# Viasat/nhd

Hardware: AMD Instinct MI355X
Metric: pod-placement filter-and-score throughput (pod x node fit-and-score evaluations/s; placement decisions/s under commit semantics in mode_b) (higher is better)
Workload: dtype u64 bitmaps + int32 table look-ups (f64 NIC arithmetic in the request digest)

## Files before the change

nhd_amd/csrc/set_states.h:

```cpp
#pragma once
#include "winner_map.h"

#include <unordered_map>
#include <vector>

namespace nhdfit {

struct SetStates {
    const uint64_t* info;
    const uint32_t* next;
    const uint32_t* asc;
    uint32_t n;
};

NHD_HD uint32_t st_key(uint64_t w, uint32_t j) { return (uint32_t)(w >> (3 * j)) & 7u; }
NHD_HD uint32_t st_count(uint64_t w) { return (uint32_t)(w >> 24) & 15u; }
NHD_HD uint32_t st_pick(uint64_t w) { return (uint32_t)(w >> 28) & 7u; }
NHD_HD uint32_t st_present(uint64_t w) { return (uint32_t)(w >> 32) & 0xFFu; }

NHD_HD uint32_t st_intersect(const SetStates& T, uint32_t a, uint32_t b) {
    const uint64_t wa = T.info[a], wb = T.info[b];
    const bool swap = st_count(wb) > st_count(wa);
    const uint64_t iter = swap ? wa : wb;
    const uint32_t probe = st_present(swap ? wb : wa);
    uint32_t out = 0;
    for (uint32_t j = 0; j < st_count(iter); ++j) {
        const uint32_t k = st_key(iter, j);
        if (probe >> k & 1) out = T.next[out * 8 + k];
    }
    return out;
}

NHD_HD uint32_t choose_g3(const SetStates& T, const AscEntry* asc, uint32_t sg_mask, uint32_t sc_mask, uint32_t nic_codes) {
    sg_mask &= 0xFFu; sc_mask &= 0xFFFFu; nic_codes &= 0xFFu;
    const uint32_t sgS = T.asc[sg_mask], cS = T.asc[nic_codes];
    const SmallSet sc = ss_from_asc(asc, 4, 2, sc_mask);
    const uint64_t wsg = T.info[sgS];
    uint32_t a = 0, b = 0;
    for (uint32_t j = 0; j < st_count(wsg); ++j) a = T.next[a * 8 + st_key(wsg, j)];
    for (int i = ss_next(sc, 0); i >= 0; i = ss_next(sc, i + 1)) b = T.next[b * 8 + ((uint32_t)ss_key(sc, i) >> 1)];
    const uint32_t abc = st_intersect(T, st_intersect(T, a, b), cS);
    const uint64_t wabc = T.info[abc];
    if (st_count(wabc) == 0) return 0;
    const uint32_t gcode = st_count(wabc) < st_count(wsg) ? st_pick(wabc) : st_pick(wsg);
    int ccode = -1;
    for (int i = ss_next(sc, 0); i >= 0 && ccode < 0; i = ss_next(sc, i + 1)) {
        const int k = ss_key(sc, i);
        if ((uint32_t)(k >> 1) == gcode) ccode = k;
    }
    return choose_result_word(ccode >= 0, gcode, ccode);
}

inline void build_set_states(std::vector<uint64_t>& info, std::vector<uint32_t>& next, std::vector<uint32_t>& asc) {
    struct Key {
        uint32_t used; int mask; uint64_t k0, k1;
        bool operator==(const Key& o) const { return used == o.used && mask == o.mask && k0 == o.k0 && k1 == o.k1; }
    };
    struct Hash {
        size_t operator()(const Key& k) const {
            uint64_t h = k.used * 0x9E3779B97F4A7C15ull ^ (uint64_t)k.mask;
            h = (h ^ k.k0) * 0xC2B2AE3D27D4EB4Full;
            h = (h ^ k.k1) * 0x165667B19E3779F9ull;
            return (size_t)(h ^ (h >> 29));
        }
    };
    std::unordered_map<Key, uint32_t, Hash> ids;
    std::vector<SmallSet> sets;
    auto intern = [&](const SmallSet& s) -> uint32_t {
        const Key key{s.used, s.mask, s.k0, s.k1};
        auto it = ids.find(key);
        if (it != ids.end()) return it->second;
        const uint32_t id = (uint32_t)sets.size();
        ids.emplace(key, id);
        sets.push_back(s);
        return id;
    };
    intern(ss_make(3, 2));
    next.clear();
    for (uint32_t s = 0; s < sets.size(); ++s) {
        for (int k = 0; k < 8; ++k) {
            const SmallSet cur = sets[s];
            const uint32_t t = (cur.present >> k & 1) ? s : intern(ss_add(cur, k));
            next.push_back(t);
        }
    }
    info.resize(sets.size());
    for (uint32_t s = 0; s < sets.size(); ++s) {
        const SmallSet& x = sets[s];
        uint64_t w = 0;
        uint32_t j = 0;
        for (int i = ss_next(x, 0); i >= 0; i = ss_next(x, i + 1)) w |= (uint64_t)ss_key(x, i) << (3 * j++);
        w |= (uint64_t)j << 24;
        if (j) w |= (uint64_t)(pick_gpu_tuple<SmallOps>(x, 3, 2) & 7) << 28;
        w |= (uint64_t)(x.present & 0xFFu) << 32;
        info[s] = w;
    }
    asc.assign(256, 0);
    for (uint32_t subset = 0; subset < 256; ++subset) {
        uint32_t s = 0;
        for (int k = 0; k < 8; ++k)
            if (subset >> k & 1) s = next[s * 8 + k];
        asc[subset] = s;
    }
// ... 4 lines not shown
```

nhd_amd/csrc/step_map.h:

```cpp
__device__ __forceinline__ bool load_winner(const MapArgs& a, uint32_t p, WinnerState& w, uint32_t& i) {
    const unsigned long long s = a.score[p];
    if (!s) return false;
    const uint64_t gi = NHDFIT_SCORE_INDEX(s);
    if (gi < a.global_base || gi >= a.global_base + a.n) return false;
    i = (uint32_t)(gi - a.global_base);
    const nhdfit_plane0 q0 = a.p0[i];
    const nhdfit_plane1 q1 = a.p1[i];
    const nhdfit_plane2 q2 = a.p2[i];
    w.d = a.det + i;
    w.U = w.d->numa_nodes;
    w.smt = (q2.flags & NHDFIT_NF_SMT) != 0;
    w.free_c[0] = popc64(q0.t0[0] & q1.t1[0]);
    w.free_c[1] = popc64(q0.t0[1] & q1.t1[1]);
    w.free_g[0] = popc32(q2.gpu_free & ~q2.gpu_numa1);
    w.free_g[1] = popc32(q2.gpu_free & q2.gpu_numa1);
    w.caps = a.caps;
    return true;
}

struct ShapeArgs {
    unsigned long long* keys;
    uint32_t* result;
    int32_t* slot_of_pod;
    uint32_t* count;
    const AscEntry* asc;
    const uint8_t* choose_tab;
    SetStates st;
};

__global__ __launch_bounds__(256) void k_build_choose(const AscEntry* asc, uint8_t* table) {
    const uint32_t e = blockIdx.x * 256 + threadIdx.x;
    if (e < kChooseEntries) table[e] = choose_entry_build(asc, e);
}

__global__ __launch_bounds__(256) void k_build_asc(AscEntry* table) {
    const uint32_t e = blockIdx.x * 256 + threadIdx.x;
    if (e >= kAscEntries) return;
    const int len = e >= kAscOffset[4] ? 4 : e >= kAscOffset[3] ? 3 : e >= kAscOffset[2] ? 2 : 1;
    table[e] = asc_entry_build(len, e - kAscOffset[len]);
}


__device__ __forceinline__ unsigned long long shfl64(unsigned long long v, int lane) {
    return ((unsigned long long)(uint32_t)__shfl((int)(v >> 32), lane, 64) << 32) | (uint32_t)__shfl((int)(uint32_t)v, lane, 64);
}

struct PaddedDet { nhdfit_detail d; uint32_t pad; };
struct StagedNode {
    int32_t node;
    uint32_t free_c[2], free_g[2];
    uint16_t sig_numa[2], sig_pci[2];
    uint32_t smt, U;
};
struct MapStage {
    PaddedReq* req; PaddedDet* det; StagedNode* w; nhdfit_mapping* map; double* caps;
};
template <int THREADS>
constexpr size_t map_lds_bytes() {
    constexpr size_t pods = THREADS / 4;
    return lds_slice(pods * sizeof(PaddedReq)) + lds_slice(pods * sizeof(PaddedDet)) + lds_slice(pods * sizeof(StagedNode)) +
           lds_slice(pods * sizeof(nhdfit_mapping)) + lds_slice(NHDFIT_MAX_CLASSES * sizeof(double));
}
constexpr uint32_t kStLdsStates = 384;
constexpr size_t kStLdsBytes = lds_slice(kStLdsStates * sizeof(uint64_t)) + lds_slice((size_t)kStLdsStates * 8 * sizeof(uint32_t)) + lds_slice(256 * sizeof(uint32_t));
template <int THREADS>
constexpr size_t map_tile_lds_bytes() { return map_lds_bytes<THREADS>() + kStLdsBytes; }
template <int THREADS>
__device__ __forceinline__ MapStage stage_winners(const MapArgs& a, uint32_t pod0, uint8_t* lds) {
    constexpr uint32_t PODS = THREADS / 4;
    MapStage s;
    s.req = carve<PaddedReq>(lds, PODS);
    s.det = carve<PaddedDet>(lds, PODS);
    s.w = carve<StagedNode>(lds, PODS);
    s.map = carve<nhdfit_mapping>(lds, PODS);
    s.caps = carve<double>(lds, NHDFIT_MAX_CLASSES);
    const uint32_t tid = threadIdx.x;
    constexpr uint32_t kParts = sizeof(nhdfit_req) / 16;
    const uint32_t live = pod0 < a.P ? (a.P - pod0 < PODS ? a.P - pod0 : PODS) : 0u;
    {
        const uint4* src = reinterpret_cast<const uint4*>(a.reqs + pod0);
        for (uint32_t c = tid; c < PODS * kParts; c += THREADS) {
            const uint32_t j = c / kParts;
            const uint4 v = j < live ? src[c] : make_uint4(0u, 0u, 0u, 0u);
            uint32_t* dst = reinterpret_cast<uint32_t*>(&s.req[j]) + (c % kParts) * 4;
            dst[0] = v.x; dst[1] = v.y; dst[2] = v.z; dst[3] = v.w;
        }
    }
    if (tid < NHDFIT_MAX_CLASSES) s.caps[tid] = a.caps[tid];
    if (tid < PODS) {
        StagedNode n;
        n.node = -1;
        n.free_c[0] = n.free_c[1] = n.free_g[0] = n.free_g[1] = 0; n.smt = 0; n.U = 1;
        n.sig_numa[0] = n.sig_numa[1] = n.sig_pci[0] = n.sig_pci[1] = 0;
        const unsigned long long sc = tid < live ? a.score[pod0 + tid] : 0ull;
        if (sc) {
            const uint64_t gi = NHDFIT_SCORE_INDEX(sc);
            if (gi >= a.global_base && gi < a.global_base + a.n) {
                const uint32_t i = (uint32_t)(gi - a.global_base);
                const nhdfit_plane0 q0 = a.p0[i];
                const nhdfit_plane1 q1 = a.p1[i];
                const nhdfit_plane2 q2 = a.p2[i];
                const nhdfit_plane3 q3 = a.p3[i];
                n.node = (int32_t)i;
                n.smt = (q2.flags & NHDFIT_NF_SMT) != 0;
                n.free_c[0] = popc64(q0.t0[0] & q1.t1[0]); n.free_c[1] = popc64(q0.t0[1] & q1.t1[1]);
                n.free_g[0] = popc32(q2.gpu_free & ~q2.gpu_numa1); n.free_g[1] = popc32(q2.gpu_free & q2.gpu_numa1);
                n.sig_numa[0] = q3.sig_numa[0]; n.sig_numa[1] = q3.sig_numa[1];
                n.sig_pci[0] = q3.sig_pci[0]; n.sig_pci[1] = q3.sig_pci[1];
            }
        }
        s.w[tid] = n;
    }
    __syncthreads();
    constexpr uint32_t kDetParts = sizeof(nhdfit_detail) / 16;
    for (uint32_t c = tid; c < PODS * kDetParts; c += THREADS) {
        const uint32_t j = c / kDetParts, part = c % kDetParts;
        const int32_t i = s.w[j].node;
        if (i >= 0) {
            const uint4 v = reinterpret_cast<const uint4*>(a.det + i)[part];
            uint32_t* dst = reinterpret_cast<uint32_t*>(&s.det[j]) + part * 4;
            dst[0] = v.x; dst[1] = v.y; dst[2] = v.z; dst[3] = v.w;
        }
    }
    __syncthreads();
    return s;
}
__device__ __forceinline__ WinnerState staged_state(const MapStage& s, uint32_t j) {
    WinnerState w;
    w.d = &s.det[j].d;
    w.U = s.det[j].d.numa_nodes;
    w.smt = s.w[j].smt != 0;
    w.free_c[0] = (int)s.w[j].free_c[0]; w.free_c[1] = (int)s.w[j].free_c[1];
    w.free_g[0] = (int)s.w[j].free_g[0]; w.free_g[1] = (int)s.w[j].free_g[1];
    w.caps = s.caps;
    return w;
}

template <int THREADS>
__device__ __forceinline__ void role_shapes(const MapArgs& a, const ShapeArgs& h, uint32_t blk, uint8_t* lds) {
    constexpr uint32_t PODS = THREADS / 4;
    const uint32_t pod0 = blk * PODS;
    const MapStage st = stage_winners<THREADS>(a, pod0, lds);
    if (threadIdx.x >= PODS) return;
    const uint32_t j = threadIdx.x, p = pod0 + j, tile = p >> 6, lane = threadIdx.x & 63;
    if (tile * 64 >= a.P) return;
    int32_t slot = -1;
    unsigned long long key = 0;
    const nhdfit_req& rq = st.req[j].r;
    if (p < a.P && rq.n_groups <= 3 && st.w[j].node >= 0) {
        const WinnerState w = staged_state(st, j);
        nhdfit_plane3 q3;
        q3.groups = 0;
        q3.sig_numa[0] = st.w[j].sig_numa[0]; q3.sig_numa[1] = st.w[j].sig_numa[1];
        q3.sig_pci[0] = st.w[j].sig_pci[0]; q3.sig_pci[1] = st.w[j].sig_pci[1];
        const uint32_t bits = nic_assignment_bits(a.tabs + (size_t)tile * a.pitch, a.L[a.tile_wcls[tile]], lane,
                                                  rq.map_type == NHDFIT_MAP_PCI, q3);
        const uint32_t codes = nic_codes_from_table_bits(bits, (int)rq.n_groups, w.U);
        uint32_t sg, sc;
        candidate_masks(rq, w, sg, sc);
        if (sg && sc && codes) {
            if (h.choose_tab && choose_tabulated((int)rq.n_groups, w.U))
                slot = -2 - (int32_t)choose_from_table(h.choose_tab, (int)rq.n_groups, sg, sc, codes);
            else
                key = shape_key((int)rq.n_groups, w.U, sg, sc, codes);
        }
    }
    unsigned long long todo = __ballot(key != 0ull);
    uint32_t nd = 0;
    while (todo) {
        const int leader = __builtin_ctzll(todo);
        const unsigned long long k = shfl64(key, leader);
        if ((int)lane == leader) h.keys[tile * 64 + nd] = k;
        if (key == k) slot = (int32_t)(tile * 64 + nd);
        todo &= ~__ballot(key == k);
        ++nd;
    }
    if (lane == 0) h.count[tile] = nd;
    if (p < a.P) h.slot_of_pod[p] = slot;
}

__device__ __forceinline__ void role_choose(const ShapeArgs& h, uint32_t w, uint32_t waves, uint32_t tiles) {
    const uint32_t S = waves / tiles ? waves / tiles : 1u;
    if (w >= S * tiles) return;
    const uint32_t tile = w % tiles, sub = w / tiles;
    const uint32_t count = (uint32_t)__builtin_amdgcn_readfirstlane((int)h.count[tile]);
    for (uint32_t j = sub; j < count; j += S) {
        const uint32_t k = tile * 64 + j;
        const unsigned long long kv = h.keys[k];
        const unsigned long long key = ((unsigned long long)(uint32_t)__builtin_amdgcn_readfirstlane((int)(kv >> 32)) << 32) |
                                       (uint32_t)__builtin_amdgcn_readfirstlane((int)(uint32_t)kv);
        const int G = (int)(key & 3), U = (int)((key >> 2) & 1) + 1;
        uint32_t gcode = 0;
        int ccode = -1;
        if (h.st.info && G == 3 && U == 2) {
            h.result[k] = choose_g3(h.st, h.asc, (uint32_t)(key >> 3) & 0xFF, (uint32_t)(key >> 19) & 0xFFFF, (uint32_t)(key >> 11) & 0xFF);
            continue;
        }
        const bool ok = choose_tuples<SmallOps>(G, U, (uint32_t)(key >> 3) & 0xFF, (uint32_t)(key >> 19) & 0xFFFF,
                                                (uint32_t)(key >> 11) & 0xFF, gcode, ccode, h.asc);
        h.result[k] = ((uint32_t)ok << 8) | ((gcode & 7u) << 4) | ((uint32_t)ccode & 15u);
    }
}

__device__ __forceinline__ void role_choose_lanes(const ShapeArgs& h, uint32_t tile, uint32_t tiles) {
    if (tile >= tiles) return;
    const uint32_t lane = threadIdx.x & 63;
    const uint32_t count = (uint32_t)__builtin_amdgcn_readfirstlane((int)h.count[tile]);
    const uint32_t k = tile * 64 + lane;
    unsigned long long key = 0;
    bool generic = false;
    if (lane < count) {
        key = h.keys[k];
        const int G = (int)(key & 3), U = (int)((key >> 2) & 1) + 1;
        if (h.st.info && G == 3 && U == 2)
            h.result[k] = choose_g3(h.st, h.asc, (uint32_t)(key >> 3) & 0xFF, (uint32_t)(key >> 19) & 0xFFFF, (uint32_t)(key >> 11) & 0xFF);
        else
            generic = true;
    }
    unsigned long long todo = __ballot(generic);
    while (todo) {
        const int j = __builtin_ctzll(todo);
        todo &= todo - 1;
        const unsigned long long kv = shfl64(key, j);
        if (lane == 0) {
            const unsigned long long kk = ((unsigned long long)(uint32_t)__builtin_amdgcn_readfirstlane((int)(kv >> 32)) << 32) |
                                          (uint32_t)__builtin_amdgcn_readfirstlane((int)(uint32_t)kv);
            const int G = (int)(kk & 3), U = (int)((kk >> 2) & 1) + 1;
            uint32_t gcode = 0;
            int ccode = -1;
            const bool ok = choose_tuples<SmallOps>(G, U, (uint32_t)(kk >> 3) & 0xFF, (uint32_t)(kk >> 19) & 0xFFFF,
                                                    (uint32_t)(kk >> 11) & 0xFF, gcode, ccode, h.asc);
            h.result[tile * 64 + j] = ((uint32_t)ok << 8) | ((gcode & 7u) << 4) | ((uint32_t)ccode & 15u);
        }
    }
}

template <int THREADS>
__device__ __forceinline__ void role_finish(const MapArgs& a, const ShapeArgs& h, uint32_t blk, uint8_t* lds) {
    constexpr uint32_t PODS = THREADS / 4;
    const uint32_t pod0 = blk * PODS;
    const MapStage st = stage_winners<THREADS>(a, pod0, lds);
    const uint32_t j = threadIdx.x, p = pod0 + j;
    if (j < PODS) {
        nhdfit_mapping& m = st.map[j];
        memset(&m, 0, sizeof(m));
        const nhdfit_req& rq = st.req[j].r;
        if (p < a.P && rq.n_groups <= 3) {
            const int32_t slot = h.slot_of_pod[p];
            if (slot != -1) {
                const uint32_t res = slot >= 0 ? h.result[slot] : (uint32_t)(-2 - slot);
                if ((res >> 8 & 1) && st.w[j].node >= 0) finish_mapping(rq, staged_state(st, j), (res >> 4) & 7u, (int)(res & 15u), m);
            }
        }
    }
    __syncthreads();
    const uint32_t live = pod0 < a.P ? (a.P - pod0 < PODS ? a.P - pod0 : PODS) : 0u;
    constexpr uint32_t kWords = sizeof(nhdfit_mapping) / 4;
    const uint32_t* src = reinterpret_cast<const uint32_t*>(st.map);
    uint32_t* dst = reinterpret_cast<uint32_t*>(a.out + pod0);
    for (uint32_t c = threadIdx.x; c < live * kWords; c += THREADS)
        if (st.req[c / kWords].r.n_groups <= 3) dst[c] = src[c];
}

template <int THREADS, bool LONE = false>
__device__ __forceinline__ void map_one_tile(const MapArgs& a, const ShapeArgs& h, uint32_t wcls, uint8_t* lds, const LoneMasks* lone = nullptr,
                                             uint32_t tile = 0, unsigned long long* clk = nullptr) {
    const unsigned long long t_blk = kTuning && clk ? (unsigned long long)wall_clock64() : 0ull;
    auto lap = [&](int k) { if (kTuning && clk && threadIdx.x == 0) atomicMax(&clk[k], (unsigned long long)wall_clock64() - t_blk); };
    static_assert(THREADS / 4 == kTile, "the pods of the tile are one wavefront");
    const uint32_t pod0 = tile * kTile;
    SetStates lst = h.st;
    if (h.st.info && h.st.n <= kStLdsStates) {
        uint8_t* q = lds + map_lds_bytes<THREADS>();
        uint64_t* l_info = carve<uint64_t>(q, kStLdsStates);
        uint32_t* l_next = carve<uint32_t>(q, (size_t)kStLdsStates * 8);
        uint32_t* l_asc = carve<uint32_t>(q, 256);
        for (uint32_t i = threadIdx.x; i < h.st.n; i += THREADS) l_info[i] = h.st.info[i];
        for (uint32_t i = threadIdx.x; i < h.st.n * 8; i += THREADS) l_next[i] = h.st.next[i];
        for (uint32_t i = threadIdx.x; i < 256; i += THREADS) l_asc[i] = h.st.asc[i];
        lst = SetStates{l_info, l_next, l_asc, h.st.n};
    }
    const MapStage st = stage_winners<THREADS>(a, pod0, lds);
    lap(0);
    const uint32_t j = threadIdx.x;
    if (j < (uint32_t)kTile) {
        const uint32_t lane = j;
        nhdfit_mapping& m = st.map[j];
        memset(&m, 0, sizeof(m));
        const nhdfit_req& rq = st.req[j].r;
        const bool live = pod0 + j < a.P && rq.n_groups <= 3 && st.w[j].node >= 0;
        int32_t slot = -1;
        unsigned long long key = 0;
        if (live) {
            const WinnerState w = staged_state(st, j);
            nhdfit_plane3 q3;
            q3.groups = 0;
            q3.sig_numa[0] = st.w[j].sig_numa[0]; q3.sig_numa[1] = st.w[j].sig_numa[1];
            q3.sig_pci[0] = st.w[j].sig_pci[0]; q3.sig_pci[1] = st.w[j].sig_pci[1];
            uint32_t bits;
            if constexpr (LONE) bits = lone_nic_bits(*lone, rq.map_type == NHDFIT_MAP_PCI, q3);
            else bits = nic_assignment_bits(a.tabs + (size_t)tile * a.pitch, a.L[wcls], lane, rq.map_type == NHDFIT_MAP_PCI, q3);
            const uint32_t codes = nic_codes_from_table_bits(bits, (int)rq.n_groups, w.U);
            uint32_t sg, sc;
            candidate_masks(rq, w, sg, sc);
            if (sg && sc && codes) {
                if (h.choose_tab && choose_tabulated((int)rq.n_groups, w.U))
                    slot = -2 - (int32_t)choose_from_table(h.choose_tab, (int)rq.n_groups, sg, sc, codes);
                else
                    key = shape_key((int)rq.n_groups, w.U, sg, sc, codes);
            }
        }
        lap(1);
        unsigned long long todo = __ballot(key != 0ull), mine = 0;
        uint32_t nd = 0;
        while (todo) {
            const int leader = __builtin_ctzll(todo);
            const unsigned long long k = shfl64(key, leader);
            if (lane == nd) mine = k;
            if (key == k) slot = (int32_t)nd;
            todo &= ~__ballot(key == k);
            ++nd;
        }
        lap(2);
        uint32_t res = 0;
        bool generic = false;
        if (lane < nd) {
            const int G = (int)(mine & 3), U = (int)((mine >> 2) & 1) + 1;
            if (lst.info && G == 3 && U == 2)
                res = choose_g3(lst, h.asc, (uint32_t)(mine >> 3) & 0xFF, (uint32_t)(mine >> 19) & 0xFFFF, (uint32_t)(mine >> 11) & 0xFF);
            else
                generic = true;
        }
        lap(3);
        unsigned long long gtodo = __ballot(generic);
        while (gtodo) {
            const int jj = __builtin_ctzll(gtodo);
            gtodo &= gtodo - 1;
            const unsigned long long kv = shfl64(mine, jj);
            uint32_t r = 0;
            if (lane == 0) {
                const unsigned long long kk = ((unsigned long long)(uint32_t)__builtin_amdgcn_readfirstlane((int)(kv >> 32)) << 32) |
                                              (uint32_t)__builtin_amdgcn_readfirstlane((int)(uint32_t)kv);
                const int G = (int)(kk & 3), U = (int)((kk >> 2) & 1) + 1;
                uint32_t gcode = 0;
                int ccode = -1;
                const bool ok = choose_tuples<SmallOps>(G, U, (uint32_t)(kk >> 3) & 0xFF, (uint32_t)(kk >> 19) & 0xFFFF,
                                                        (uint32_t)(kk >> 11) & 0xFF, gcode, ccode, h.asc);
                r = ((uint32_t)ok << 8) | ((gcode & 7u) << 4) | ((uint32_t)ccode & 15u);
            }
            r = (uint32_t)__shfl((int)r, 0, 64);
            if ((int)lane == jj) res = r;
        }
        lap(4);
        const uint32_t got = (uint32_t)__shfl((int)res, slot >= 0 ? slot : 0, 64);
        if (live && slot != -1) {
            const uint32_t rr = slot >= 0 ? got : (uint32_t)(-2 - slot);
            if (rr >> 8 & 1) finish_mapping(rq, staged_state(st, j), (rr >> 4) & 7u, (int)(rr & 15u), m);
        }
        lap(5);
    }
    __syncthreads();
    const uint32_t livep = pod0 < a.P ? (a.P - pod0 < (uint32_t)kTile ? a.P - pod0 : (uint32_t)kTile) : 0u;
    constexpr uint32_t kWords = sizeof(nhdfit_mapping) / 4;
    const uint32_t* src = reinterpret_cast<const uint32_t*>(st.map);
    uint32_t* dst = reinterpret_cast<uint32_t*>(a.out + pod0);
    for (uint32_t c = threadIdx.x; c < livep * kWords; c += THREADS)
        if (st.req[c / kWords].r.n_groups <= 3) dst[c] = src[c];
}

constexpr int kDrainSteps = 3;
struct DrainArgs {
    uint32_t nsteps, tiles;
    MapArgs m[kDrainSteps];
    ShapeArgs h;
    unsigned long long* clk;
};
__global__ __launch_bounds__(256) void k_map_tiles(DrainArgs a) {
    extern __shared__ __align__(16) uint8_t lds_drain[];
    const uint32_t s = (uint32_t)__builtin_amdgcn_readfirstlane((int)(blockIdx.x / a.tiles)), tile = blockIdx.x - s * a.tiles;
    const MapArgs& m = a.m[s < (uint32_t)kDrainSteps ? s : 0];
    const unsigned long long t0 = kTuning && a.clk ? (unsigned long long)wall_clock64() : 0ull;
    map_one_tile<256>(m, a.h, m.tile_wcls[tile], lds_drain, nullptr, tile, kTuning ? a.clk : nullptr);
    if (kTuning && a.clk && threadIdx.x == 0) { atomicMin(&a.clk[7], t0); atomicMax(&a.clk[6], (unsigned long long)wall_clock64()); }
}
// ... 1 lines not shown
```

nhd_amd/csrc/winner_map.h:

```cpp
#pragma once
#include "fit_core.h"

namespace nhdfit {

constexpr uint64_t kXX1 = 11400714785074694791ULL;
constexpr uint64_t kXX2 = 14029467366897019727ULL;
constexpr uint64_t kXX5 = 2870177450012600261ULL;

constexpr uint64_t py_tuple_hash_calc(uint32_t code, int len) {
    uint64_t acc = kXX5;
    for (int i = 0; i < len; ++i) {
        const uint64_t lane = (code >> (len - 1 - i)) & 1u;
        acc += lane * kXX2;
        acc = (acc << 31) | (acc >> 33);
        acc *= kXX1;
    }
    acc += (uint64_t)len ^ (kXX5 ^ 3527539ULL);
    if (acc == (uint64_t)-1) return 1546275796ULL;
    return acc;
}
struct TupleHashTable { uint64_t h[6][32]; };
constexpr TupleHashTable make_tuple_hash_table() {
    TupleHashTable t{};
    for (int len = 0; len <= 5; ++len)
// ... 195 lines not shown
    s.k0 |= slot < 16 ? v : 0;
    s.k1 |= slot >= 16 ? v : 0;
    s.used |= 1u << slot;
    return s;
}
NHD_HD int ss_free_slot(uint32_t used, int mask, int len, int key) {
    const int home = home_slot(len, mask, key);
    if (!(used >> home & 1)) return home;
    const ProbeRow r = probe_row(len, mask, (uint32_t)key);
    uint64_t w = r.lo;
    for (int n = 0; n < kProbeLen; ++n) {
        if (n == 12) w = r.hi;
        const int slot = (int)(w & 31u);
        if (!(used >> slot & 1)) return slot;
        w >>= 5;
    }
    const uint64_t h = py_tuple_hash((uint32_t)key, len, 2);
    uint64_t perturb = h;
    uint32_t i = (uint32_t)(h & (uint64_t)mask);
    for (;;) {
        const int probes = (i + 9 <= (uint32_t)mask) ? 9 : 0;
        for (int j = 0; j <= probes; ++j)
            if (!(used >> (i + j) & 1)) return (int)(i + j);
        perturb >>= 5;
        i = (uint32_t)((i * 5 + 1 + perturb) & (uint64_t)mask);
    }
}
NHD_HD SmallSet ss_add(SmallSet s, int key) {
    if (s.present >> key & 1) return s;
    s = ss_put(s, ss_free_slot(s.used, s.mask, s.len, key), key);
    s.present |= 1u << key;
    s.fill++;
    if (s.fill * 5 >= s.mask * 3) {
        const SmallSet o = s;
        s.used = 0; s.mask = 31; s.k0 = s.k1 = 0;
        for (int i = ss_next(o, 0); i >= 0; i = ss_next(o, i + 1)) {
            const int k = ss_key(o, i);
            s = ss_put(s, ss_free_slot(s.used, 31, s.len, k), k);
        }
    }
    return s;
}
NHD_HD bool ss_has(SmallSet s, int key) { return (s.present >> key & 1) != 0; }

struct AscEntry { uint32_t used, pad; uint64_t k0, k1; };
constexpr uint32_t kAscOffset[5] = {0, 0, 4, 20, 276};
constexpr uint32_t kAscEntries = 276 + 65536;
NHD_HD AscEntry asc_entry_build(int len, uint32_t subset) {
    SmallSet s = ss_make(len, 2);
    for (uint32_t code = 0; code < (1u << len); ++code)
        if (subset >> code & 1) s = ss_add(s, (int)code);
    return AscEntry{s.used, 0u, s.k0, s.k1};
}
NHD_HD SmallSet ss_from_asc(const AscEntry* table, int len, int base, uint32_t subset) {
    const AscEntry e = table[kAscOffset[len] + subset];
    SmallSet s;
    s.used = e.used; s.present = subset; s.fill = popc32(subset); s.mask = s.fill >= 5 ? 31 : 7;
    s.len = len; s.base = base; s.k0 = e.k0; s.k1 = e.k1;
    return s;
}
NHD_HD SmallSet ss_intersect(SmallSet a, SmallSet b) {
    SmallSet out = ss_make(a.len, a.base);
    const bool swap = b.fill > a.fill;
    const SmallSet probe = swap ? b : a;
    const SmallSet iter = swap ? a : b;
    for (int i = ss_next(iter, 0); i >= 0; i = ss_next(iter, i + 1)) {
        const int k = ss_key(iter, i);
        if (ss_has(probe, k)) out = ss_add(out, k);
    }
    return out;
}
NHD_HD int ss_list(SmallSet s, int16_t* out) {
    int n = 0;
    for (int i = 0; i <= s.mask; ++i)
        if (s.used >> i & 1) out[n++] = (int16_t)ss_key(s, i);
    return n;
}

struct GenericOps {
    typedef PySet Set;
    NHD_HD static void init(Set& s, int, int) { ps_init(s); }
    NHD_HD static void from_subset(Set& s, const AscEntry*, int len, int base, uint32_t subset) {
        ps_init(s);
        for (uint32_t code = 0; code < 32; ++code)
            if (subset >> code & 1) ps_add(s, (int16_t)code, py_tuple_hash(code, len, base));
    }
    NHD_HD static void add(Set& s, int key, int len, int base) { ps_add(s, (int16_t)key, py_tuple_hash((uint32_t)key, len, base)); }
    NHD_HD static void isect(const Set& a, const Set& b, Set& o) { ps_intersect(a, b, o); }
    NHD_HD static int list(const Set& s, int16_t* o) { return ps_list(s, o); }
    NHD_HD static int size(const Set& s) { return s.fill; }
    NHD_HD static int next(const Set& s, int from) { for (int i = from; i <= s.mask; ++i) if (s.key[i] >= 0) return i; return -1; }
    NHD_HD static int key_at(const Set& s, int slot) { return s.key[slot]; }
};
struct SmallOps {
    typedef SmallSet Set;
    NHD_HD static void init(Set& s, int len, int base) { s = ss_make(len, base); }
    NHD_HD static void from_subset(Set& s, const AscEntry* table, int len, int base, uint32_t subset) {
        if (table) { s = ss_from_asc(table, len, base, subset); return; }
        s = ss_make(len, base);
        for (uint32_t code = 0; code < (1u << len); ++code)
            if (subset >> code & 1) s = ss_add(s, (int)code);
    }
    NHD_HD static void add(Set& s, int key, int, int) { s = ss_add(s, key); }
    NHD_HD static void isect(const Set& a, const Set& b, Set& o) { o = ss_intersect(a, b); }
    NHD_HD static int list(const Set& s, int16_t* o) { return ss_list(s, o); }
    NHD_HD static int size(const Set& s) { return s.fill; }
    NHD_HD static int next(const Set& s, int from) { return ss_next(s, from); }
    NHD_HD static int key_at(const Set& s, int slot) { return ss_key(s, slot); }
};

struct WinnerState {
    int U;
    bool smt;
    int free_c[2], free_g[2];
    const nhdfit_detail* d;
    const double* caps;
};

NHD_HD int tup_digit(uint32_t code, int len, int U, int i) {
    (void)U;
    return (int)((code >> (len - 1 - i)) & 1u);
}

NHD_HD uint32_t ipow(int b, int e) { return b == 1 ? 1u : 1u << e; }

NHD_HD uint32_t nib_get(uint32_t v, int i) { return (v >> (4 * i)) & 15u; }
NHD_HD uint32_t nib_set(uint32_t v, int i, uint32_t x) { return (v & ~(15u << (4 * i))) | (x << (4 * i)); }

NHD_HD bool first_nic_choice_plain(const nhdfit_req& r, const WinnerState& w, uint32_t gcode, bool pci, int8_t nic_idx[kMaxG]) {
    const int G = (int)r.n_groups;
    uint32_t order = 0, numa = 0;
    int n = 0;
    for (int u = 0; u < w.U; ++u)
        for (int g = 0; g < G; ++g)
            if (tup_digit(gcode, G, w.U, g) == u) { order = nib_set(order, n, (uint32_t)g); numa |= (uint32_t)u << g; ++n; }
    for (int g = 0; g < G; ++g)
        if (w.d->nic_cnt[(numa >> g) & 1] == 0) return false;
    uint32_t pick = 0;
    for (;;) {
        bool ok = true;
        for (int g = 0; g < G && ok; ++g) {
            const uint32_t u = (numa >> g) & 1, k = nib_get(pick, g);
            bool first_on_nic = true;
            for (int h = 0; h < g; ++h)
                if (((numa >> h) & 1) == u && nib_get(pick, h) == k) first_on_nic = false;
            if (!first_on_nic) continue;
            double rx = w.caps[w.d->nic_cls[u][k]], tx = rx;
            for (int h = g; h < G; ++h)
                if (((numa >> h) & 1) == u && nib_get(pick, h) == k) { rx = rx - r.rx[h]; tx = tx - r.tx[h]; }
            if (rx < 0 || tx < 0) ok = false;
        }
        if (ok && pci) {
            for (int g = 0; g < G && ok; ++g) {
                const uint32_t s = w.d->nic_sw[(numa >> g) & 1][nib_get(pick, g)];
                uint32_t cnt = 0;
                for (int h = 0; h < G; ++h)
                    if (w.d->nic_sw[(numa >> h) & 1][nib_get(pick, h)] == s) ++cnt;
                if (cnt > w.d->sw_free[s]) ok = false;
            }
        }
        if (ok) {
            for (int g = 0; g < G; ++g) nic_idx[g] = (int8_t)nib_get(pick, g);
            return true;
        }
        int pos = G - 1;
        while (pos >= 0) {
            const int g = (int)nib_get(order, pos);
            const uint32_t v = nib_get(pick, g) + 1;
            if (v < w.d->nic_cnt[(numa >> g) & 1]) { pick = nib_set(pick, g, v); break; }
            pick = nib_set(pick, g, 0);
            --pos;
        }
        if (pos < 0) return false;
    }
}

NHD_HD bool first_nic_choice(const nhdfit_req& r, const WinnerState& w, uint32_t gcode, bool pci, int8_t nic_idx[kMaxG]) {
    const int G = (int)r.n_groups;
    uint32_t order = 0, numa = 0;
    int n = 0;
    for (int u = 0; u < w.U; ++u)
        for (int g = 0; g < G; ++g)
            if (tup_digit(gcode, G, w.U, g) == u) { order = nib_set(order, n, (uint32_t)g); numa |= (uint32_t)u << g; ++n; }
    for (int g = 0; g < G; ++g)
        if (w.d->nic_cnt[(numa >> g) & 1] == 0) return false;
    for (int g = 0; g < G; ++g)
        if (!(r.rx[g] >= 0) || !(r.tx[g] >= 0)) return first_nic_choice_plain(r, w, gcode, pci, nic_idx);
    uint32_t pick = 0;
    auto prefix_ok = [&](int pos) {
        const int g = (int)nib_get(order, pos);
        const uint32_t u = (numa >> g) & 1, k = nib_get(pick, g);
        double rx = w.caps[w.d->nic_cls[u][k]], tx = rx;
        for (int q = 0; q <= pos; ++q) {
            const int h = (int)nib_get(order, q);
            if (((numa >> h) & 1) == u && nib_get(pick, h) == k) { rx = rx - r.rx[h]; tx = tx - r.tx[h]; }
        }
        if (rx < 0 || tx < 0) return false;
        if (pci) {
            const uint32_t sw = w.d->nic_sw[u][k];
            uint32_t cnt = 0;
            for (int q = 0; q <= pos; ++q) {
                const int h = (int)nib_get(order, q);
                if (w.d->nic_sw[(numa >> h) & 1][nib_get(pick, h)] == sw) ++cnt;
            }
            if (cnt > w.d->sw_free[sw]) return false;
        }
        return true;
    };
    int pos = 0;
    for (;;) {
        if (prefix_ok(pos)) {
            if (pos == G - 1) {
                for (int g = 0; g < G; ++g) nic_idx[g] = (int8_t)nib_get(pick, g);
                return true;
            }
            ++pos;
            continue;
        }
        for (;;) {
            const int g = (int)nib_get(order, pos);
            const uint32_t v = nib_get(pick, g) + 1;
            if (v < w.d->nic_cnt[(numa >> g) & 1]) { pick = nib_set(pick, g, v); break; }
            pick = nib_set(pick, g, 0);
            if (--pos < 0) return false;
        }
    }
}

NHD_HD uint32_t nic_codes_from_table_bits(uint32_t bits, int G, int U) {
    if (U == 1) return bits & 1u;
    uint32_t out = 0;
    for (uint32_t p = 0; p < (1u << G); ++p) {
        if (!(bits >> p & 1)) continue;
        uint32_t code = 0;
        for (int i = 0; i < G; ++i) code |= (p >> i & 1u) << (G - 1 - i);
        out |= 1u << code;
    }
    return out;
}

template <class Ops>
NHD_HD int pick_gpu_tuple(const typename Ops::Set& gset, int G, int U) {
    int best = -1, best_spread = -1;
    for (int i = Ops::next(gset, 0); i >= 0; i = Ops::next(gset, i + 1)) {
        const int k = Ops::key_at(gset, i);
        int ones = 0;
        for (int g = 0; g < G; ++g) ones += tup_digit((uint32_t)k, G, U, g);
        const int zeros = G - ones;
        const int spread = U == 1 ? 0 : (ones > zeros ? ones - zeros : zeros - ones);
        if (spread > best_spread) { best_spread = spread; best = k; }
    }
    return best;
}

template <class Ops>
NHD_HD bool choose_tuples(int G, int U, uint32_t sg_mask, uint32_t sc_mask, uint32_t nic_codes, uint32_t& gcode, int& ccode,
                          const AscEntry* asc = nullptr) {
    typedef typename Ops::Set Set;
    const uint32_t nG = ipow(U, G), nC = ipow(U, G + 1);
    Set sg, sc;
    Ops::from_subset(sg, asc, G, U, sg_mask & ((1u << nG) - 1u));
    Ops::from_subset(sc, asc, G + 1, U, sc_mask & (nC >= 32 ? ~0u : (1u << nC) - 1u));
    Set a, b, c, ab, abc;
    Ops::init(a, G, U); Ops::init(b, G, U);
    for (int i = Ops::next(sg, 0); i >= 0; i = Ops::next(sg, i + 1)) Ops::add(a, Ops::key_at(sg, i), G, U);
    for (int i = Ops::next(sc, 0); i >= 0; i = Ops::next(sc, i + 1)) Ops::add(b, Ops::key_at(sc, i) >> (U - 1), G, U);
    Ops::from_subset(c, asc, G, U, nic_codes & ((1u << nG) - 1u));
    Ops::isect(a, b, ab);
    Ops::isect(ab, c, abc);
    if (Ops::size(abc) == 0) return false;
    gcode = (uint32_t)(Ops::size(abc) < Ops::size(sg) ? pick_gpu_tuple<Ops>(abc, G, U) : pick_gpu_tuple<Ops>(sg, G, U));
    ccode = -1;
    for (int i = Ops::next(sc, 0); i >= 0 && ccode < 0; i = Ops::next(sc, i + 1)) {
        const int k = Ops::key_at(sc, i);
        if ((uint32_t)(k >> (U - 1)) == gcode) ccode = k;
    }
// ... 101 lines not shown
```

Baseline: 15760 billion.

## Stage NIC bits and detail records in parallel, pack NIC walk fields into registers

Detail records are now loaded by all four thread quarters directly, without waiting on a barrier for the staged node index. NIC assignment bits are computed during staging and stored in the staged node, replacing the saved signature fields. The AscEntry used by choose_g3 is prefetched per pod and passed to the leader lane with shuffles. The NIC backtracking walk packs classes, switches and switch-free counts into 64-bit nibble registers and uses a placed-mask with fixed-length unrolled loops, which should cut LDS reads and loop overhead at the cost of more registers and extra shuffle work.

```diff
diff --git a/nhd_amd/csrc/set_states.h b/nhd_amd/csrc/set_states.h
--- a/nhd_amd/csrc/set_states.h
+++ b/nhd_amd/csrc/set_states.h
@@ -31,14 +31,18 @@
     return out;
 }
 
-NHD_HD uint32_t choose_g3(const SetStates& T, const AscEntry* asc, uint32_t sg_mask, uint32_t sc_mask, uint32_t nic_codes) {
-    sg_mask &= 0xFFu; sc_mask &= 0xFFFFu; nic_codes &= 0xFFu;
+NHD_HD uint32_t choose_g3_set(const SetStates& T, uint32_t sg_mask, SmallSet sc, uint32_t nic_codes) {
+    sg_mask &= 0xFFu; nic_codes &= 0xFFu;
     const uint32_t sgS = T.asc[sg_mask], cS = T.asc[nic_codes];
-    const SmallSet sc = ss_from_asc(asc, 4, 2, sc_mask);
     const uint64_t wsg = T.info[sgS];
-    uint32_t a = 0, b = 0;
+    uint32_t a = 0, b = 0, in_b = 0;
     for (uint32_t j = 0; j < st_count(wsg); ++j) a = T.next[a * 8 + st_key(wsg, j)];
-    for (int i = ss_next(sc, 0); i >= 0; i = ss_next(sc, i + 1)) b = T.next[b * 8 + ((uint32_t)ss_key(sc, i) >> 1)];
+    for (int i = ss_next(sc, 0); i >= 0; i = ss_next(sc, i + 1)) {
+        const uint32_t k = (uint32_t)ss_key(sc, i) >> 1;
+        if (in_b >> k & 1) continue;
+        in_b |= 1u << k;
+        b = T.next[b * 8 + k];
+    }
     const uint32_t abc = st_intersect(T, st_intersect(T, a, b), cS);
     const uint64_t wabc = T.info[abc];
     if (st_count(wabc) == 0) return 0;
@@ -49,6 +53,9 @@
         if ((uint32_t)(k >> 1) == gcode) ccode = k;
     }
     return choose_result_word(ccode >= 0, gcode, ccode);
+}
+NHD_HD uint32_t choose_g3(const SetStates& T, const AscEntry* asc, uint32_t sg_mask, uint32_t sc_mask, uint32_t nic_codes) {
+    return choose_g3_set(T, sg_mask, ss_from_asc(asc, 4, 2, sc_mask & 0xFFFFu), nic_codes);
 }
 
 inline void build_set_states(std::vector<uint64_t>& info, std::vector<uint32_t>& next, std::vector<uint32_t>& asc) {
diff --git a/nhd_amd/csrc/step_map.h b/nhd_amd/csrc/step_map.h
--- a/nhd_amd/csrc/step_map.h
+++ b/nhd_amd/csrc/step_map.h
@@ -49,11 +49,17 @@
 struct StagedNode {
     int32_t node;
     uint32_t free_c[2], free_g[2];
-    uint16_t sig_numa[2], sig_pci[2];
-    uint32_t smt, U;
+    uint32_t smt;
+    uint32_t bits;
+    uint32_t pad[2];
 };
 struct MapStage {
     PaddedReq* req; PaddedDet* det; StagedNode* w; nhdfit_mapping* map; double* caps;
+};
+enum StageNic : int {
+    kStageNoNic = 0,
+    kStageTileNic = 1,
+    kStageLoneNic = 2,
 };
 template <int THREADS>
 constexpr size_t map_lds_bytes() {
@@ -65,9 +71,11 @@
 constexpr size_t kStLdsBytes = lds_slice(kStLdsStates * sizeof(uint64_t)) + lds_slice((size_t)kStLdsStates * 8 * sizeof(uint32_t)) + lds_slice(256 * sizeof(uint32_t));
 template <int THREADS>
 constexpr size_t map_tile_lds_bytes() { return map_lds_bytes<THREADS>() + kStLdsBytes; }
-template <int THREADS>
-__device__ __forceinline__ MapStage stage_winners(const MapArgs& a, uint32_t pod0, uint8_t* lds) {
+template <int THREADS, int NIC>
+__device__ __forceinline__ MapStage stage_winners(const MapArgs& a, uint32_t pod0, uint8_t* lds, uint32_t wcls = ~0u, const LoneMasks* lone = nullptr) {
     constexpr uint32_t PODS = THREADS / 4;
+    constexpr uint32_t kDetParts = sizeof(nhdfit_detail) / 16;
+    static_assert(kDetParts == 8 && THREADS == 4 * PODS, "a quarter of the threads per two 16-byte parts of a detail record");
     MapStage s;
     s.req = carve<PaddedReq>(lds, PODS);
     s.det = carve<PaddedDet>(lds, PODS);
@@ -87,40 +95,45 @@
         }
     }
     if (tid < NHDFIT_MAX_CLASSES) s.caps[tid] = a.caps[tid];
-    if (tid < PODS) {
+    const uint32_t j = tid % PODS, quarter = tid / PODS, p = pod0 + j;
+    const unsigned long long sc = j < live ? a.score[p] : 0ull;
+    bool pci = false;
+    uint32_t wc = wcls;
+    if (NIC != kStageNoNic && quarter == 0 && j < live) {
+        pci = a.reqs[p].map_type == NHDFIT_MAP_PCI;
+        if (NIC == kStageTileNic && wcls == ~0u) wc = a.tile_wcls[p >> 6];
+    }
+    int32_t node = -1;
+    if (sc) {
+        const uint64_t gi = NHDFIT_SCORE_INDEX(sc);
+        if (gi >= a.global_base && gi < a.global_base + a.n) node = (int32_t)(gi - a.global_base);
+    }
+    if (node >= 0) {
+        const uint4* src = reinterpret_cast<const uint4*>(a.det + node) + quarter * 2;
+        const uint4 v0 = src[0], v1 = src[1];
+        uint32_t* dst = reinterpret_cast<uint32_t*>(&s.det[j]) + quarter * 8;
+        dst[0] = v0.x; dst[1] = v0.y; dst[2] = v0.z; dst[3] = v0.w;
+        dst[4] = v1.x; dst[5] = v1.y; dst[6] = v1.z; dst[7] = v1.w;
+    }
+    if (quarter == 0) {
         StagedNode n;
-        n.node = -1;
-        n.free_c[0] = n.free_c[1] = n.free_g[0] = n.free_g[1] = 0; n.smt = 0; n.U = 1;
-        n.sig_numa[0] = n.sig_numa[1] = n.sig_pci[0] = n.sig_pci[1] = 0;
-        const unsigned long long sc = tid < live ? a.score[pod0 + tid] : 0ull;
-        if (sc) {
-            const uint64_t gi = NHDFIT_SCORE_INDEX(sc);
-            if (gi >= a.global_base && gi < a.global_base + a.n) {
-                const uint32_t i = (uint32_t)(gi - a.global_base);
-                const nhdfit_plane0 q0 = a.p0[i];
-                const nhdfit_plane1 q1 = a.p1[i];
-                const nhdfit_plane2 q2 = a.p2[i];
-                const nhdfit_plane3 q3 = a.p3[i];
-                n.node = (int32_t)i;
-                n.smt = (q2.flags & NHDFIT_NF_SMT) != 0;
-                n.free_c[0] = popc64(q0.t0[0] & q1.t1[0]); n.free_c[1] = popc64(q0.t0[1] & q1.t1[1]);
-                n.free_g[0] = popc32(q2.gpu_free & ~q2.gpu_numa1); n.free_g[1] = popc32(q2.gpu_free & q2.gpu_numa1);
-                n.sig_numa[0] = q3.sig_numa[0]; n.sig_numa[1] = q3.sig_numa[1];
-                n.sig_pci[0] = q3.sig_pci[0]; n.sig_pci[1] = q3.sig_pci[1];
-            }
-        }
-        s.w[tid] = n;
-    }
-    __syncthreads();
-    constexpr uint32_t kDetParts = sizeof(nhdfit_detail) / 16;
-    for (uint32_t c = tid; c < PODS * kDetParts; c += THREADS) {
-        const uint32_t j = c / kDetParts, part = c % kDetParts;
-        const int32_t i = s.w[j].node;
-        if (i >= 0) {
-            const uint4 v = reinterpret_cast<const uint4*>(a.det + i)[part];
-            uint32_t* dst = reinterpret_cast<uint32_t*>(&s.det[j]) + part * 4;
-            dst[0] = v.x; dst[1] = v.y; dst[2] = v.z; dst[3] = v.w;
-        }
+        n.node = node;
+        n.free_c[0] = n.free_c[1] = n.free_g[0] = n.free_g[1] = 0; n.smt = 0; n.bits = 0;
+        n.pad[0] = n.pad[1] = 0;
+        if (node >= 0) {
+            const nhdfit_plane0 q0 = a.p0[node];
+            const nhdfit_plane1 q1 = a.p1[node];
+            const nhdfit_plane2 q2 = a.p2[node];
+            const nhdfit_plane3 q3 = a.p3[node];
+            n.smt = (q2.flags & NHDFIT_NF_SMT) != 0;
+            n.free_c[0] = popc64(q0.t0[0] & q1.t1[0]); n.free_c[1] = popc64(q0.t0[1] & q1.t1[1]);
+            n.free_g[0] = popc32(q2.gpu_free & ~q2.gpu_numa1); n.free_g[1] = popc32(q2.gpu_free & q2.gpu_numa1);
+            if constexpr (NIC == kStageTileNic)
+                n.bits = nic_assignment_bits(a.tabs + (size_t)(p >> 6) * a.pitch, a.L[wc], p & 63, pci, q3);
+            else if constexpr (NIC == kStageLoneNic)
+                n.bits = lone_nic_bits(*lone, pci, q3);
+        }
+        s.w[j] = n;
     }
     __syncthreads();
     return s;
@@ -140,7 +153,7 @@
 __device__ __forceinline__ void role_shapes(const MapArgs& a, const ShapeArgs& h, uint32_t blk, uint8_t* lds) {
     constexpr uint32_t PODS = THREADS / 4;
     const uint32_t pod0 = blk * PODS;
-    const MapStage st = stage_winners<THREADS>(a, pod0, lds);
+    const MapStage st = stage_winners<THREADS, kStageTileNic>(a, pod0, lds);
     if (threadIdx.x >= PODS) return;
     const uint32_t j = threadIdx.x, p = pod0 + j, tile = p >> 6, lane = threadIdx.x & 63;
     if (tile * 64 >= a.P) return;
@@ -149,13 +162,7 @@
     const nhdfit_req& rq = st.req[j].r;
     if (p < a.P && rq.n_groups <= 3 && st.w[j].node >= 0) {
         const WinnerState w = staged_state(st, j);
-        nhdfit_plane3 q3;
-        q3.groups = 0;
-        q3.sig_numa[0] = st.w[j].sig_numa[0]; q3.sig_numa[1] = st.w[j].sig_numa[1];
-        q3.sig_pci[0] = st.w[j].sig_pci[0]; q3.sig_pci[1] = st.w[j].sig_pci[1];
-        const uint32_t bits = nic_assignment_bits(a.tabs + (size_t)tile * a.pitch, a.L[a.tile_wcls[tile]], lane,
-                                                  rq.map_type == NHDFIT_MAP_PCI, q3);
-        const uint32_t codes = nic_codes_from_table_bits(bits, (int)rq.n_groups, w.U);
+        const uint32_t codes = nic_codes_from_table_bits(st.w[j].bits, (int)rq.n_groups, w.U);
         uint32_t sg, sc;
         candidate_masks(rq, w, sg, sc);
         if (sg && sc && codes) {
@@ -239,7 +246,7 @@
 __device__ __forceinline__ void role_finish(const MapArgs& a, const ShapeArgs& h, uint32_t blk, uint8_t* lds) {
     constexpr uint32_t PODS = THREADS / 4;
     const uint32_t pod0 = blk * PODS;
-    const MapStage st = stage_winners<THREADS>(a, pod0, lds);
+    const MapStage st = stage_winners<THREADS, kStageNoNic>(a, pod0, lds);
     const uint32_t j = threadIdx.x, p = pod0 + j;
     if (j < PODS) {
         nhdfit_mapping& m = st.map[j];
@@ -269,18 +276,20 @@
     auto lap = [&](int k) { if (kTuning && clk && threadIdx.x == 0) atomicMax(&clk[k], (unsigned long long)wall_clock64() - t_blk); };
     static_assert(THREADS / 4 == kTile, "the pods of the tile are one wavefront");
     const uint32_t pod0 = tile * kTile;
-    SetStates lst = h.st;
-    if (h.st.info && h.st.n <= kStLdsStates) {
-        uint8_t* q = lds + map_lds_bytes<THREADS>();
-        uint64_t* l_info = carve<uint64_t>(q, kStLdsStates);
-        uint32_t* l_next = carve<uint32_t>(q, (size_t)kStLdsStates * 8);
-        uint32_t* l_asc = carve<uint32_t>(q, 256);
+    const bool use_st = h.st.info && h.st.n <= kStLdsStates;
+    uint8_t* q = lds + map_lds_bytes<THREADS>();
+    uint64_t* l_info = carve<uint64_t>(q, kStLdsStates);
+    uint32_t* l_next = carve<uint32_t>(q, (size_t)kStLdsStates * 8);
+    uint32_t* l_asc = carve<uint32_t>(q, 256);
+    if (use_st) {
         for (uint32_t i = threadIdx.x; i < h.st.n; i += THREADS) l_info[i] = h.st.info[i];
         for (uint32_t i = threadIdx.x; i < h.st.n * 8; i += THREADS) l_next[i] = h.st.next[i];
         for (uint32_t i = threadIdx.x; i < 256; i += THREADS) l_asc[i] = h.st.asc[i];
-        lst = SetStates{l_info, l_next, l_asc, h.st.n};
-    }
-    const MapStage st = stage_winners<THREADS>(a, pod0, lds);
+    }
+    const SetStates lst{l_info, l_next, l_asc, h.st.n};
+    MapStage st;
+    if constexpr (LONE) st = stage_winners<THREADS, kStageLoneNic>(a, pod0, lds, wcls, lone);
+    else st = stage_winners<THREADS, kStageTileNic>(a, pod0, lds, wcls);
     lap(0);
     const uint32_t j = threadIdx.x;
     if (j < (uint32_t)kTile) {
@@ -291,16 +300,10 @@
         const bool live = pod0 + j < a.P && rq.n_groups <= 3 && st.w[j].node >= 0;
         int32_t slot = -1;
         unsigned long long key = 0;
+        AscEntry pre{0u, 0u, 0ull, 0ull};
         if (live) {
             const WinnerState w = staged_state(st, j);
-            nhdfit_plane3 q3;
-            q3.groups = 0;
-            q3.sig_numa[0] = st.w[j].sig_numa[0]; q3.sig_numa[1] = st.w[j].sig_numa[1];
-            q3.sig_pci[0] = st.w[j].sig_pci[0]; q3.sig_pci[1] = st.w[j].sig_pci[1];
-            uint32_t bits;
-            if constexpr (LONE) bits = lone_nic_bits(*lone, rq.map_type == NHDFIT_MAP_PCI, q3);
-            else bits = nic_assignment_bits(a.tabs + (size_t)tile * a.pitch, a.L[wcls], lane, rq.map_type == NHDFIT_MAP_PCI, q3);
-            const uint32_t codes = nic_codes_from_table_bits(bits, (int)rq.n_groups, w.U);
+            const uint32_t codes = nic_codes_from_table_bits(st.w[j].bits, (int)rq.n_groups, w.U);
             uint32_t sg, sc;
             candidate_masks(rq, w, sg, sc);
             if (sg && sc && codes) {
@@ -308,15 +311,16 @@
                     slot = -2 - (int32_t)choose_from_table(h.choose_tab, (int)rq.n_groups, sg, sc, codes);
                 else
                     key = shape_key((int)rq.n_groups, w.U, sg, sc, codes);
+                if (use_st && rq.n_groups == 3 && w.U == 2) pre = h.asc[kAscOffset[4] + (sc & 0xFFFFu)];
             }
         }
         lap(1);
         unsigned long long todo = __ballot(key != 0ull), mine = 0;
-        uint32_t nd = 0;
+        uint32_t nd = 0, from = 0;
         while (todo) {
             const int leader = __builtin_ctzll(todo);
             const unsigned long long k = shfl64(key, leader);
-            if (lane == nd) mine = k;
+            if (lane == nd) { mine = k; from = (uint32_t)leader; }
             if (key == k) slot = (int32_t)nd;
             todo &= ~__ballot(key == k);
             ++nd;
@@ -324,12 +328,21 @@
         lap(2);
         uint32_t res = 0;
         bool generic = false;
-        if (lane < nd) {
-            const int G = (int)(mine & 3), U = (int)((mine >> 2) & 1) + 1;
-            if (lst.info && G == 3 && U == 2)
-                res = choose_g3(lst, h.asc, (uint32_t)(mine >> 3) & 0xFF, (uint32_t)(mine >> 19) & 0xFFFF, (uint32_t)(mine >> 11) & 0xFF);
-            else
-                generic = true;
+        {
+            AscEntry e;
+            e.used = (uint32_t)__shfl((int)pre.used, (int)from, 64);
+            e.pad = 0u;
+            e.k0 = shfl64(pre.k0, (int)from);
+            e.k1 = shfl64(pre.k1, (int)from);
+            if (lane < nd) {
+                const int G = (int)(mine & 3), U = (int)((mine >> 2) & 1) + 1;
+                if (use_st && G == 3 && U == 2) {
+                    const uint32_t scm = (uint32_t)(mine >> 19) & 0xFFFF;
+                    res = choose_g3_set(lst, (uint32_t)(mine >> 3) & 0xFF, ss_from_entry(e, 4, 2, scm), (uint32_t)(mine >> 11) & 0xFF);
+                } else {
+                    generic = true;
+                }
+            }
         }
         lap(3);
         unsigned long long gtodo = __ballot(generic);
diff --git a/nhd_amd/csrc/winner_map.h b/nhd_amd/csrc/winner_map.h
--- a/nhd_amd/csrc/winner_map.h
+++ b/nhd_amd/csrc/winner_map.h
@@ -271,12 +271,14 @@
         if (subset >> code & 1) s = ss_add(s, (int)code);
     return AscEntry{s.used, 0u, s.k0, s.k1};
 }
-NHD_HD SmallSet ss_from_asc(const AscEntry* table, int len, int base, uint32_t subset) {
-    const AscEntry e = table[kAscOffset[len] + subset];
+NHD_HD SmallSet ss_from_entry(const AscEntry& e, int len, int base, uint32_t subset) {
     SmallSet s;
     s.used = e.used; s.present = subset; s.fill = popc32(subset); s.mask = s.fill >= 5 ? 31 : 7;
     s.len = len; s.base = base; s.k0 = e.k0; s.k1 = e.k1;
     return s;
+}
+NHD_HD SmallSet ss_from_asc(const AscEntry* table, int len, int base, uint32_t subset) {
+    return ss_from_entry(table[kAscOffset[len] + subset], len, base, subset);
 }
 NHD_HD SmallSet ss_intersect(SmallSet a, SmallSet b) {
     SmallSet out = ss_make(a.len, a.base);
@@ -346,15 +348,63 @@
 NHD_HD uint32_t nib_get(uint32_t v, int i) { return (v >> (4 * i)) & 15u; }
 NHD_HD uint32_t nib_set(uint32_t v, int i, uint32_t x) { return (v & ~(15u << (4 * i))) | (x << (4 * i)); }
 
-NHD_HD bool first_nic_choice_plain(const nhdfit_req& r, const WinnerState& w, uint32_t gcode, bool pci, int8_t nic_idx[kMaxG]) {
-    const int G = (int)r.n_groups;
-    uint32_t order = 0, numa = 0;
+struct NicWalk {
+    uint64_t cls0, cls1, sw0, sw1, sw_free;
+    uint32_t cnt0, cnt1;
+    const double* rx; const double* tx;
+};
+NHD_HD uint32_t ld32_aligned(const void* p) {
+    uint32_t x;
+    __builtin_memcpy(&x, __builtin_assume_aligned(p, 4), 4);
+    return x;
+}
+NHD_HD uint64_t nibbles16(const uint8_t* b) {
+    uint64_t v = 0;
+#pragma unroll
+    for (int i = 0; i < 4; ++i) {
+        const uint32_t x = ld32_aligned(b + 4 * i);
+        v |= (uint64_t)((x & 0xFu) | (x >> 4 & 0xF0u) | (x >> 8 & 0xF00u) | (x >> 12 & 0xF000u)) << (16 * i);
+    }
+    return v;
+}
+NHD_HD NicWalk nic_walk_fields(const nhdfit_req& r, const nhdfit_detail* d) {
+    static_assert(__builtin_offsetof(nhdfit_detail, sw_free) == 2 && __builtin_offsetof(nhdfit_detail, nic_cls) == 16 && __builtin_offsetof(nhdfit_detail, nic_sw) == 48 &&
+                  NHDFIT_MAX_SWITCHES == 14 && NHDFIT_MAX_NICS_PER_NUMA == 16, "record layout the nibble packing assumes");
+    NicWalk f;
+    const uint8_t* b = reinterpret_cast<const uint8_t*>(d);
+    f.cls0 = nibbles16(b + 16); f.cls1 = nibbles16(b + 32);
+    f.sw0 = nibbles16(b + 48); f.sw1 = nibbles16(b + 64);
+    uint32_t head[4];
+#pragma unroll
+    for (int i = 0; i < 4; ++i) head[i] = ld32_aligned(b + 4 * i);
+    f.cnt0 = head[0] & 0xFFu; f.cnt1 = head[0] >> 8 & 0xFFu;
+    f.sw_free = 0;
+#pragma unroll
+    for (int s = 0; s < NHDFIT_MAX_SWITCHES; ++s) {
+        const uint32_t v = head[(s + 2) / 4] >> (8 * ((s + 2) % 4)) & 0xFFu;
+        f.sw_free |= (uint64_t)(v < 15u ? v : 15u) << (4 * s);
+    }
+    f.rx = r.rx; f.tx = r.tx;
+    return f;
+}
+NHD_HD uint64_t pick64(uint64_t v0, uint64_t v1, uint32_t u) { return v0 ^ ((v0 ^ v1) & (0ull - (uint64_t)(u & 1u))); }
+NHD_HD uint32_t nw_cls(const NicWalk& f, uint32_t u, uint32_t k) { return (uint32_t)(pick64(f.cls0, f.cls1, u) >> (4 * k)) & 15u; }
+NHD_HD uint32_t nw_sw(const NicWalk& f, uint32_t u, uint32_t k) { return (uint32_t)(pick64(f.sw0, f.sw1, u) >> (4 * k)) & 15u; }
+NHD_HD uint32_t nw_cnt(const NicWalk& f, uint32_t u) { return (uint32_t)pick64(f.cnt0, f.cnt1, u); }
+NHD_HD uint32_t nw_sw_free(const NicWalk& f, uint32_t s) { return (uint32_t)(f.sw_free >> (4 * s)) & 15u; }
+
+NHD_HD bool nic_walk_order(const NicWalk f, int G, int U, uint32_t gcode, uint32_t& order, uint32_t& numa) {
+    order = numa = 0;
     int n = 0;
-    for (int u = 0; u < w.U; ++u)
+    for (int u = 0; u < U; ++u)
         for (int g = 0; g < G; ++g)
-            if (tup_digit(gcode, G, w.U, g) == u) { order = nib_set(order, n, (uint32_t)g); numa |= (uint32_t)u << g; ++n; }
+            if (tup_digit(gcode, G, U, g) == u) { order = nib_set(order, n, (uint32_t)g); numa |= (uint32_t)u << g; ++n; }
     for (int g = 0; g < G; ++g)
-        if (w.d->nic_cnt[(numa >> g) & 1] == 0) return false;
+        if (nw_cnt(f, numa >> g) == 0) return false;
+    return true;
+}
+
+NHD_HD bool nic_walk_plain(const NicWalk f, const double* caps, int G, uint32_t order, uint32_t numa, bool pci, int8_t nic_idx[kMaxG]) {
     uint32_t pick = 0;
     for (;;) {
         bool ok = true;
@@ -364,18 +414,20 @@
             for (int h = 0; h < g; ++h)
                 if (((numa >> h) & 1) == u && nib_get(pick, h) == k) first_on_nic = false;
             if (!first_on_nic) continue;
-            double rx = w.caps[w.d->nic_cls[u][k]], tx = rx;
-            for (int h = g; h < G; ++h)
-                if (((numa >> h) & 1) == u && nib_get(pick, h) == k) { rx = rx - r.rx[h]; tx = tx - r.tx[h]; }
+            double rx = caps[nw_cls(f, u, k)], tx = rx;
+#pragma unroll
+            for (int h = 0; h < kMaxG; ++h)
+                if (h >= g && h < G && ((numa >> h) & 1) == u && nib_get(pick, h) == k) { rx = rx - f.rx[h]; tx = tx - f.tx[h]; }
             if (rx < 0 || tx < 0) ok = false;
         }
         if (ok && pci) {
             for (int g = 0; g < G && ok; ++g) {
-                const uint32_t s = w.d->nic_sw[(numa >> g) & 1][nib_get(pick, g)];
+                const uint32_t s = nw_sw(f, (numa >> g) & 1, nib_get(pick, g));
                 uint32_t cnt = 0;
-                for (int h = 0; h < G; ++h)
-                    if (w.d->nic_sw[(numa >> h) & 1][nib_get(pick, h)] == s) ++cnt;
-                if (cnt > w.d->sw_free[s]) ok = false;
+#pragma unroll
+                for (int h = 0; h < kMaxG; ++h)
+                    if (h < G && nw_sw(f, (numa >> h) & 1, nib_get(pick, h)) == s) ++cnt;
+                if (cnt > nw_sw_free(f, s)) ok = false;
             }
         }
         if (ok) {
@@ -386,7 +438,7 @@
         while (pos >= 0) {
             const int g = (int)nib_get(order, pos);
             const uint32_t v = nib_get(pick, g) + 1;
-            if (v < w.d->nic_cnt[(numa >> g) & 1]) { pick = nib_set(pick, g, v); break; }
+            if (v < nw_cnt(f, numa >> g)) { pick = nib_set(pick, g, v); break; }
             pick = nib_set(pick, g, 0);
             --pos;
         }
@@ -394,39 +446,46 @@
     }
 }
 
+NHD_HD bool first_nic_choice_plain(const nhdfit_req& r, const WinnerState& w, uint32_t gcode, bool pci, int8_t nic_idx[kMaxG]) {
+    const int G = (int)r.n_groups;
+    const NicWalk f = nic_walk_fields(r, w.d);
+    uint32_t order, numa;
+    if (!nic_walk_order(f, G, w.U, gcode, order, numa)) return false;
+    return nic_walk_plain(f, w.caps, G, order, numa, pci, nic_idx);
+}
+
 NHD_HD bool first_nic_choice(const nhdfit_req& r, const WinnerState& w, uint32_t gcode, bool pci, int8_t nic_idx[kMaxG]) {
     const int G = (int)r.n_groups;
-    uint32_t order = 0, numa = 0;
-    int n = 0;
-    for (int u = 0; u < w.U; ++u)
-        for (int g = 0; g < G; ++g)
-            if (tup_digit(gcode, G, w.U, g) == u) { order = nib_set(order, n, (uint32_t)g); numa |= (uint32_t)u << g; ++n; }
-    for (int g = 0; g < G; ++g)
-        if (w.d->nic_cnt[(numa >> g) & 1] == 0) return false;
-    for (int g = 0; g < G; ++g)
-        if (!(r.rx[g] >= 0) || !(r.tx[g] >= 0)) return first_nic_choice_plain(r, w, gcode, pci, nic_idx);
+    const NicWalk f = nic_walk_fields(r, w.d);
+    uint32_t order, numa;
+    if (!nic_walk_order(f, G, w.U, gcode, order, numa)) return false;
+    bool monotone = true;
+#pragma unroll
+    for (int g = 0; g < kMaxG; ++g)
+        if (g < G && (!(f.rx[g] >= 0) || !(f.tx[g] >= 0))) monotone = false;
+    if (!monotone) return nic_walk_plain(f, w.caps, G, order, numa, pci, nic_idx);
     uint32_t pick = 0;
+    uint32_t placed = 0;
     auto prefix_ok = [&](int pos) {
         const int g = (int)nib_get(order, pos);
         const uint32_t u = (numa >> g) & 1, k = nib_get(pick, g);
-        double rx = w.caps[w.d->nic_cls[u][k]], tx = rx;
-        for (int q = 0; q <= pos; ++q) {
-            const int h = (int)nib_get(order, q);
-            if (((numa >> h) & 1) == u && nib_get(pick, h) == k) { rx = rx - r.rx[h]; tx = tx - r.tx[h]; }
-        }
+        double rx = w.caps[nw_cls(f, u, k)], tx = rx;
+#pragma unroll
+        for (int h = 0; h < kMaxG; ++h)
+            if ((placed >> h & 1) && ((numa >> h) & 1) == u && nib_get(pick, h) == k) { rx = rx - f.rx[h]; tx = tx - f.tx[h]; }
         if (rx < 0 || tx < 0) return false;
         if (pci) {
-            const uint32_t sw = w.d->nic_sw[u][k];
+            const uint32_t sw = nw_sw(f, u, k);
             uint32_t cnt = 0;
-            for (int q = 0; q <= pos; ++q) {
-                const int h = (int)nib_get(order, q);
-                if (w.d->nic_sw[(numa >> h) & 1][nib_get(pick, h)] == sw) ++cnt;
-            }
-            if (cnt > w.d->sw_free[sw]) return false;
+#pragma unroll
+            for (int h = 0; h < kMaxG; ++h)
+                if ((placed >> h & 1) && nw_sw(f, (numa >> h) & 1, nib_get(pick, h)) == sw) ++cnt;
+            if (cnt > nw_sw_free(f, sw)) return false;
         }
         return true;
     };
     int pos = 0;
+    placed = 1u << nib_get(order, 0);
     for (;;) {
         if (prefix_ok(pos)) {
             if (pos == G - 1) {
@@ -434,13 +493,15 @@
                 return true;
             }
             ++pos;
+            placed |= 1u << nib_get(order, pos);
             continue;
         }
         for (;;) {
             const int g = (int)nib_get(order, pos);
             const uint32_t v = nib_get(pick, g) + 1;
-            if (v < w.d->nic_cnt[(numa >> g) & 1]) { pick = nib_set(pick, g, v); break; }
+            if (v < nw_cnt(f, numa >> g)) { pick = nib_set(pick, g, v); break; }
             pick = nib_set(pick, g, 0);
+            placed &= ~(1u << g);
             if (--pos < 0) return false;
         }
     }
```

Result: faster. 16580 billion, median of 6 (+5.2%).
